# nyu-systems/Grendel-GS

Measured on AMD Instinct MI355X. Metric: training iters/sec (fwd+bwd), higher is better.
Workload: dtype f32

## Files before the change

grendel-gs_amd/csrc/composite.hip:

```cpp
#include "common.h"

namespace {

constexpr float LOG2E = 1.4426950408889634f;
constexpr float ALPHA_MIN = 1.0f / 255.0f;
constexpr float T_STOP = 0.0001f;

__device__ unsigned long long g_walked[2];

#ifdef GSR_STATS
__device__ unsigned long long g_stats[8];
#define GSR_STAT(i, v) do { const unsigned long long sv__ = (unsigned long long)(v); if (lane == 0) atomicAdd(&g_stats[i], sv__); } while (0)
#else
#define GSR_STAT(i, v) do { } while (0)
#endif

struct Entry {
    float x, y;
    float a2, b2, c2;
    float o;
    bool relevant;
};

#ifndef GSR_NO_LOG2O
#define GSR_LOG2O 1
#endif
__device__ __forceinline__ float entry_exponent(const float4 q0, const float4 q1, float dx, float dy) {
#ifdef GSR_LOG2O
    return fmaf(fmaf(q0.z, dx, q0.w * dy), dx, fmaf(q1.x * dy, dy, q1.y));
#else
    return (q0.z * dx + q0.w * dy) * dx + q1.x * dy * dy;
#endif
}
__device__ __forceinline__ float entry_alpha_raw(const float4 q1, float pe) {
#ifdef GSR_LOG2O
    return __builtin_amdgcn_exp2f(pe);
#else
    return q1.y * __builtin_amdgcn_exp2f(pe);
#endif
}
__device__ __forceinline__ bool entry_power_ok(const float4 q1, float pe) {
#ifdef GSR_LOG2O
    return pe <= q1.y;
#else
    return pe <= 0.f;
#endif
}

__device__ __forceinline__ float entry_opacity_term(float o) {
#ifdef GSR_LOG2O
    return __log2f(o);
#else
    return o;
#endif
}

__device__ __forceinline__ Entry load_entry(bool have, uint32_t id, const float2 *__restrict__ means2D,
                                            const float4 *__restrict__ conic_opacity, float qx0, float qy0) {
    Entry e;
    e.x = e.y = e.a2 = e.b2 = e.c2 = e.o = 0.f;
    e.relevant = false;
    if (have) {
        const float2 xy = means2D[id];
        const float4 co = conic_opacity[id];
        e.x = xy.x;
        e.y = xy.y;
        e.a2 = -0.5f * LOG2E * co.x;
        e.b2 = -LOG2E * co.y;
        e.c2 = -0.5f * LOG2E * co.z;
        e.o = entry_opacity_term(co.w);
        e.relevant = gsr_can_touch_box(xy, co, qx0, qy0, qx0 + 7.0f, qy0 + 7.0f);
    }
    return e;
}


typedef float v2f __attribute__((ext_vector_type(2)));
constexpr int PREC = 20;
struct PairRec {
    v2f x, y, a2, b2, c2, o, r, g, b;
};
__device__ __forceinline__ void pair_store(float *__restrict__ slab, int pos, const Entry &e, float r, float g, float b) {
    float *rec = slab + (pos >> 1) * PREC + (pos & 1);
    rec[0] = e.x;  rec[2] = e.y;  rec[4] = e.a2;  rec[6] = e.b2;  rec[8] = e.c2;
    rec[10] = e.o; rec[12] = r;   rec[14] = g;    rec[16] = b;
}
__device__ __forceinline__ void pair_store_last(float *__restrict__ slab, int pos, int last) {
    slab[(pos >> 1) * PREC + 18 + (pos & 1)] = __int_as_float(last);
}
__device__ __forceinline__ PairRec pair_load_last(const float *__restrict__ slab, int pair, int &la, int &lb) {
    const float4 *q = reinterpret_cast<const float4 *>(slab + pair * PREC);
    const float4 q0 = q[0], q1 = q[1], q2 = q[2], q3 = q[3], q4 = q[4];
    PairRec p;
    p.x = v2f{q0.x, q0.y};  p.y = v2f{q0.z, q0.w};  p.a2 = v2f{q1.x, q1.y};  p.b2 = v2f{q1.z, q1.w};
    p.c2 = v2f{q2.x, q2.y}; p.o = v2f{q2.z, q2.w};  p.r = v2f{q3.x, q3.y};   p.g = v2f{q3.z, q3.w};
    p.b = v2f{q4.x, q4.y};
    la = __float_as_int(q4.z);
    lb = __float_as_int(q4.w);
    asm("" : "+v"(la), "+v"(lb));
    return p;
}
#ifdef GSR_LOG2O
#define GSR_PAD_O (-__builtin_inff())
#else
#define GSR_PAD_O 0.f
#endif
__device__ __forceinline__ PairRec pair_load(const float *__restrict__ slab, int pair) {
    const float4 *q = reinterpret_cast<const float4 *>(slab + pair * PREC);
    const float4 q0 = q[0], q1 = q[1], q2 = q[2], q3 = q[3];
    const float2 q4 = *reinterpret_cast<const float2 *>(q + 4);
    PairRec p;
    p.x = v2f{q0.x, q0.y};  p.y = v2f{q0.z, q0.w};  p.a2 = v2f{q1.x, q1.y};  p.b2 = v2f{q1.z, q1.w};
    p.c2 = v2f{q2.x, q2.y}; p.o = v2f{q2.z, q2.w};  p.r = v2f{q3.x, q3.y};   p.g = v2f{q3.z, q3.w};
    p.b = v2f{q4.x, q4.y};
    return p;
}
__device__ __forceinline__ v2f pair_exponent(const PairRec &p, float pxf, float pyf) {
    const v2f dx = p.x - pxf, dy = p.y - pyf;
    return __builtin_elementwise_fma(__builtin_elementwise_fma(p.a2, dx, p.b2 * dy), dx,
                                     __builtin_elementwise_fma(p.c2 * dy, dy, p.o));
}

__device__ __forceinline__ int composite_tile_of_block(const int2 *__restrict__ ranges, int gx, int tiles) {
    const int2 hull = ranges[tiles];
    const int gy = tiles / gx;
    if (hull.x < 0 || hull.y > gy || hull.x >= hull.y) return gsr_xcd_span_of_block(blockIdx.x, tiles);
    return gsr_xcd_span_of_block_band(blockIdx.x, tiles, hull.x * gx, (hull.y - hull.x) * gx);
}

struct RawEntry {
    float2 xy;
    float4 co;
    float r, g, b;
};
__device__ __forceinline__ RawEntry load_raw(bool have, uint32_t id, const float2 *__restrict__ means2D,
                                             const float4 *__restrict__ conic_opacity, const float *__restrict__ rgb) {
    RawEntry e;
    e.xy = make_float2(0.f, 0.f);
    e.co = make_float4(0.f, 0.f, 0.f, 0.f);
    e.r = e.g = e.b = 0.f;
    if (have) {
        e.xy = means2D[id];
        e.co = conic_opacity[id];
        e.r = rgb[3 * (size_t)id];
        e.g = rgb[3 * (size_t)id + 1];
        e.b = rgb[3 * (size_t)id + 2];
    }
    return e;
}

#ifndef GSR_SEG_LEN
#define GSR_SEG_LEN 256
#endif
#ifndef GSR_SEG_MAXJ
#define GSR_SEG_MAXJ 16
#endif
constexpr int SEG_LEN = GSR_SEG_LEN;
constexpr int SEG_MAXJ = GSR_SEG_MAXJ;
static_assert(SEG_LEN % 64 == 0 && (SEG_LEN & (SEG_LEN - 1)) == 0 && SEG_MAXJ <= 31,
              "segment geometry: K8 finds boundaries with c & (SEG_LEN - 1), so SEG_LEN is a power of two");
constexpr int SEG_WORKERS = 1024;
constexpr int SEG_SLOT_FLOATS = 7 * 256;
struct SegWs {
    uint32_t *hdr;
    uint32_t *queue;
    int32_t *seg_slot;
    float *ckpt;
    uint32_t cap;
};
__host__ __device__ inline size_t seg_ws_bytes(int tiles, uint32_t cap) {
    return 64 + sizeof(uint32_t) * (size_t)cap + sizeof(int32_t) * (size_t)tiles * SEG_MAXJ + sizeof(float) * SEG_SLOT_FLOATS * (size_t)cap;
}
inline SegWs seg_ws_of(void *ws, int tiles, uint32_t cap) {
    SegWs w{};
    if (!ws) return w;
    char *b = reinterpret_cast<char *>(ws);
    w.hdr = reinterpret_cast<uint32_t *>(b);
    w.queue = reinterpret_cast<uint32_t *>(b + 64);
    w.seg_slot = reinterpret_cast<int32_t *>(b + 64 + sizeof(uint32_t) * (size_t)cap);
    w.ckpt = reinterpret_cast<float *>(b + 64 + sizeof(uint32_t) * (size_t)cap + sizeof(int32_t) * (size_t)tiles * SEG_MAXJ);
    w.cap = cap;
    return w;
}
constexpr uint32_t SEG_CAP = 8192;

__device__ __forceinline__ int k8_checkpoint(const SegWs &seg, int *s_slot, int tile, int c, int lane,
                                                       int wave, float T, float c0, float c1, float c2) {
    const int j = c / SEG_LEN - 1;
    int slot = 0;
    if (lane == 0) {
        int v = atomicCAS(&s_slot[j], -1, -2);
        if (v == -1) {
            const uint32_t k = atomicAdd(seg.hdr, 1u);
            v = k < seg.cap ? (int)k : -3;
            if (v >= 0) {
                seg.queue[k] = (uint32_t)tile * 32u + (uint32_t)(j + 1);
                seg.seg_slot[(size_t)tile * SEG_MAXJ + j] = v;
            }
            __hip_atomic_store(&s_slot[j], v, __ATOMIC_RELEASE, __HIP_MEMORY_SCOPE_WORKGROUP);
        } else {
            while (v == -2) v = __hip_atomic_load(&s_slot[j], __ATOMIC_ACQUIRE, __HIP_MEMORY_SCOPE_WORKGROUP);
        }
        slot = v;
    }
    slot = __builtin_amdgcn_readfirstlane(slot);
    if (slot >= 0) {
        float *ck = seg.ckpt + (size_t)slot * SEG_SLOT_FLOATS + wave * 64 + lane;
        ck[0] = T;
        ck[256] = c0;
        ck[512] = c1;
        ck[768] = c2;
    }
    return slot;
}

template <bool SEG, bool BAND>
__global__ void __launch_bounds__(256, SEG ? 6 : (BAND ? 7 : 8))
composite_forward_kernel(int W, int H, int gx, const int2 *__restrict__ ranges,
                         const uint32_t *__restrict__ point_list, const float2 *__restrict__ means2D,
                         const float4 *__restrict__ conic_opacity, const float *__restrict__ rgb,
                         const uint8_t *__restrict__ compute_locally, const float *__restrict__ bg,
                         float *__restrict__ out_color, float *__restrict__ final_T, int32_t *__restrict__ n_contrib,
                         const SegWs seg, int band_first, int band_tiles, uint4 *__restrict__ zero16,
                         size_t zero16_n) {
    const size_t HW = (size_t)H * W;
    for (size_t i = (size_t)blockIdx.x * 256 + threadIdx.x; i < zero16_n; i += (size_t)gridDim.x * 256)
        zero16[i] = make_uint4(0u, 0u, 0u, 0u);
    int tile;
    bool idle = false;
    if (BAND) {
        if (band_first < 0) {
            const int gy = (H + GSR_BLOCK_Y - 1) / GSR_BLOCK_Y;
            int2 hull = ranges[gx * gy];
            if (hull.x < 0 || hull.y > gy || hull.x >= hull.y) hull = make_int2(0, 0);
            band_first = hull.x * gx;
            band_tiles = min((hull.y - hull.x) * gx, band_tiles);
            idle = (int)blockIdx.x >= band_tiles;
        }
        tile = band_first + (idle ? 0 : gsr_xcd_span_of_block(blockIdx.x, band_tiles));
    } else {
        tile = composite_tile_of_block(ranges, gx, (int)gridDim.x);
    }
    auto clear_outside = [&]() {
        if (!BAND) return;
        const size_t n0 = (size_t)min(H, (band_first / gx) * GSR_BLOCK_Y) * W;
        const size_t p1 = (size_t)min(H, ((band_first + band_tiles) / gx) * GSR_BLOCK_Y) * W;
        const size_t nout = n0 + (HW - p1);
        for (size_t i = (size_t)blockIdx.x * 256 + threadIdx.x; i < nout; i += (size_t)gridDim.x * 256) {
            const size_t q = i < n0 ? i : p1 + (i - n0);
            out_color[q] = 0.f;
            out_color[HW + q] = 0.f;
            out_color[2 * HW + q] = 0.f;
            final_T[q] = 1.f;
            n_contrib[q] = 0;
        }
    };
    if (idle) {
        clear_outside();
        return;
    }
    const int lane = threadIdx.x & 63, wave = threadIdx.x >> 6;
    const int tx = tile % gx, ty = tile / gx;
    const int qx0 = tx * GSR_BLOCK_X + (wave & 1) * 8, qy0 = ty * GSR_BLOCK_Y + (wave >> 1) * 8;
    const int px = qx0 + (lane & 7), py = qy0 + (lane >> 3);
    const bool inside = px < W && py < H;
    const size_t pid = (size_t)py * W + px;

    if (!compute_locally[tile]) {
        if (inside) {
            out_color[pid] = 0.f;
            out_color[HW + pid] = 0.f;
            out_color[2 * HW + pid] = 0.f;
            final_T[pid] = 1.f;
            n_contrib[pid] = 0;
        }
        clear_outside();
        return;
    }
    const int2 range = ranges[tile];
    const int n = range.y - range.x;
    const float pxf = (float)px, pyf = (float)py;

    float T = 1.0f, C0 = 0.f, C1 = 0.f, C2 = 0.f;
    int last = 0;
    bool done = !inside;
    __shared__ __attribute__((aligned(16))) float slab[4][32 * PREC];
    __shared__ int s_walk[2];
    __shared__ int s_slot[SEG_MAXJ];
    if (threadIdx.x < 2) s_walk[threadIdx.x] = 0;
    if (SEG && threadIdx.x < SEG_MAXJ) {
        s_slot[threadIdx.x] = -1;
        if (seg.seg_slot) seg.seg_slot[(size_t)tile * SEG_MAXJ + threadIdx.x] = -1;
    }
    __syncthreads();
    v2f A0 = {0.f, 0.f}, A1 = {0.f, 0.f}, A2 = {0.f, 0.f};
    v2f B0 = {0.f, 0.f}, B1 = {0.f, 0.f}, B2 = {0.f, 0.f};
    int nstored = 0;
    float *wslab = slab[wave];
    int walked = 0;

    for (int c = 0; c < n; c += 64) {
        if (__all(done)) break;
        if (SEG && seg.seg_slot && c > 0 && (c & (SEG_LEN - 1)) == 0 && c <= SEG_LEN * SEG_MAXJ) {
            if (k8_checkpoint(seg, s_slot, tile, c, lane, wave, T, B0.x + B0.y, B1.x + B1.y, B2.x + B2.y) >= 0) {
                B0 = B1 = B2 = v2f{0.f, 0.f};
                nstored = c / SEG_LEN;
            }
        }
        walked = c + 64;
        const bool have = c + lane < n;
        const uint32_t id = have ? point_list[range.x + c + lane] : 0u;
        const Entry e = load_entry(have, id, means2D, conic_opacity, (float)qx0, (float)qy0);
        float r = 0.f, g = 0.f, b = 0.f;
        if (e.relevant) {
            r = rgb[3 * (size_t)id];
            g = rgb[3 * (size_t)id + 1];
            b = rgb[3 * (size_t)id + 2];
        }
        unsigned long long m = __ballot(e.relevant);
        GSR_STAT(0, __popcll(__ballot(have)));
        GSR_STAT(1, __popcll(m));
        const int nrel = __popcll(m);
#ifdef GSR_ABL_K8_MASKWALK
        if (e.relevant) pair_store(wslab, __popcll(m & ((1ull << lane) - 1ull)), e, r, g, b);
        {
            const int pad = (-nrel) & 3, slot = nrel + lane / 9;
            if (lane < 9 * pad) wslab[(slot >> 1) * PREC + 2 * (lane % 9) + (slot & 1)] = 0.f;
        }
#else
        if (e.relevant) {
            const int pos = __popcll(m & ((1ull << lane) - 1ull));
            pair_store(wslab, pos, e, r, g, b);
            pair_store_last(wslab, pos, c + lane + 1);
        }
        {
            const int pad = (-nrel) & 3, slot = nrel + lane / 10, f = lane % 10;
            if (lane < 10 * pad) wslab[(slot >> 1) * PREC + 2 * f + (slot & 1)] = f == 5 ? GSR_PAD_O : 0.f;
        }
#endif
        for (int p0 = 0; p0 < nrel; p0 += 4) {
            float al[4];
            bool ok[4];
            int kk[4];
            v2f cr[2], cg[2], cb[2];
#pragma unroll
            for (int h = 0; h < 2; h++) {
#ifdef GSR_ABL_K8_MASKWALK
                const PairRec pr = pair_load(wslab, (p0 >> 1) + h);
#else
                const PairRec pr = pair_load_last(wslab, (p0 >> 1) + h, kk[2 * h], kk[2 * h + 1]);
#endif
                const v2f pe = pair_exponent(pr, pxf, pyf);
                cr[h] = pr.r;
                cg[h] = pr.g;
                cb[h] = pr.b;
#pragma unroll
                for (int u = 0; u < 2; u++) {
#ifdef GSR_ABL_K8_MASKWALK
                    const bool live = m != 0;
                    kk[2 * h + u] = c + (live ? __builtin_ctzll(m) : 0) + 1;
                    m &= m - 1;
#else
                    const bool live = true;
#endif
                    const float pe1 = u ? pe.y : pe.x, lo = u ? pr.o.y : pr.o.x;
                    al[2 * h + u] = fminf(0.99f, __builtin_amdgcn_exp2f(pe1));
                    ok[2 * h + u] = live && pe1 <= lo && al[2 * h + u] >= ALPHA_MIN;
                }
            }
            float wv[4];
#pragma unroll
            for (int u = 0; u < 4; u++) {
                const float w0 = al[u] * T;
                const float test_T = T - w0;
                const bool take = !done && ok[u];
                const bool stop = take && __float_as_int(test_T) < __float_as_int(T_STOP);
                done = done || stop;
                const bool blend = take && !stop;
                wv[u] = blend ? w0 : 0.f;
                T = blend ? test_T : T;
                last = blend ? kk[u] : last;
            }
#pragma unroll
            for (int h = 0; h < 2; h++) {
                const v2f w2 = {wv[2 * h], wv[2 * h + 1]};
                A0 = __builtin_elementwise_fma(cr[h], w2, A0);
                A1 = __builtin_elementwise_fma(cg[h], w2, A1);
                A2 = __builtin_elementwise_fma(cb[h], w2, A2);
                if (SEG) {
                    B0 = __builtin_elementwise_fma(cr[h], w2, B0);
                    B1 = __builtin_elementwise_fma(cg[h], w2, B1);
                    B2 = __builtin_elementwise_fma(cb[h], w2, B2);
                }
            }
            if (__all(done)) break;
        }
    }
    if (lane == 0) {
        atomicMax(&s_walk[0], walked < n ? walked : n);
        if (atomicAdd(&s_walk[1], 1) == 3) atomicAdd(&g_walked[0], (unsigned long long)s_walk[0]);
    }
    C0 = A0.x + A0.y;
    C1 = A1.x + A1.y;
    C2 = A2.x + A2.y;
    if (SEG && nstored > 0) {
        float r0 = B0.x + B0.y, r1 = B1.x + B1.y, r2 = B2.x + B2.y;
        for (int j = nstored - 1; j >= 0; j--) {
            float *ck = seg.ckpt + (size_t)s_slot[j] * SEG_SLOT_FLOATS + wave * 64 + lane;
            ck[1024] = r0;
            ck[1280] = r1;
            ck[1536] = r2;
            r0 += ck[256];
            r1 += ck[512];
            r2 += ck[768];
        }
    }
    if (inside) {
        out_color[pid] = C0 + T * bg[0];
        out_color[HW + pid] = C1 + T * bg[1];
        out_color[2 * HW + pid] = C2 + T * bg[2];
        final_T[pid] = T;
        n_contrib[pid] = last;
    }
    clear_outside();
}

typedef float f32x4 __attribute__((ext_vector_type(4)));

constexpr int MB = 8;
constexpr int MSTR = 66;

__device__ __forceinline__ void
composite_backward_segment(const int tile, const int sidx, int W, int H, int gx, const int2 *__restrict__ ranges,
                           const uint32_t *__restrict__ point_list, const float2 *__restrict__ means2D,
                           const float4 *__restrict__ conic_opacity, const float *__restrict__ rgb,
                           const uint8_t *__restrict__ compute_locally, const float *__restrict__ bg,
                           const float *__restrict__ final_T, const int32_t *__restrict__ n_contrib,
                           const float *__restrict__ dL_dpixels, double *__restrict__ dL_record,
                           const SegWs &seg, uint8_t *__restrict__ touched) {
    if (!compute_locally[tile]) return;
    const int lane = threadIdx.x & 63, wave = threadIdx.x >> 6;
    const int tx = tile % gx, ty = tile / gx;
    const int qx0 = tx * GSR_BLOCK_X + (wave & 1) * 8, qy0 = ty * GSR_BLOCK_Y + (wave >> 1) * 8;
    const int px = qx0 + (lane & 7), py = qy0 + (lane >> 3);
    const bool inside = px < W && py < H;
    const size_t pid = (size_t)py * W + px;
    const size_t HW = (size_t)H * W;
    const int2 range = ranges[tile];
    const float pxf = (float)px, pyf = (float)py;

    const int c_lo = sidx * SEG_LEN;
    int end_slot = -1;
    if (seg.seg_slot && sidx < SEG_MAXJ) end_slot = seg.seg_slot[(size_t)tile * SEG_MAXJ + sidx];
    const int c_hi = end_slot >= 0 ? c_lo + SEG_LEN : 0x7fffffff;
    const float T_final = inside ? final_T[pid] : 0.f;
    const int last = inside ? n_contrib[pid] : 0;
    float g0 = 0.f, g1 = 0.f, g2 = 0.f;
    if (inside) {
        g0 = dL_dpixels[pid];
        g1 = dL_dpixels[HW + pid];
        g2 = dL_dpixels[2 * HW + pid];
    }
    const float tb = T_final * (bg[0] * g0 + bg[1] * g1 + bg[2] * g2);
    const float ddelx_dx = 0.5f * W, ddely_dy = 0.5f * H;

    __shared__ float2 smat[4][MB * MSTR];
    __shared__ float sacc[4][64 * 9];
    __shared__ __attribute__((aligned(16))) float slab[4][32 * PREC];
    __shared__ float fslab[64 * 7];
    __shared__ float sout[64 * 10];
    __shared__ int s_wmax[4];
    int wmax = min(last, c_hi);
#pragma unroll
    for (int d = 32; d >= 1; d >>= 1) wmax = max(wmax, __shfl_xor(wmax, d, 64));
    if (wmax <= c_lo) wmax = 0;
    if (lane == 0) s_wmax[wave] = wmax;
    for (int i = threadIdx.x; i < 4 * 64 * 9; i += 256) (&sacc[0][0])[i] = 0.f;
    __syncthreads();
    const int bmax = max(max(s_wmax[0], s_wmax[1]), max(s_wmax[2], s_wmax[3]));
    if (bmax == 0) return;
    if (threadIdx.x == 0) atomicAdd(&g_walked[1], (unsigned long long)(bmax - c_lo));
    int wbest = 0;
#pragma unroll
    for (int w = 1; w < 4; w++)
        if (s_wmax[w] > s_wmax[wbest]) wbest = w;

    const int kq = lane >> 4, j = lane & 15;
    float Bop[16];
    {
        const bool isg = j >= 6 && j < 9;
        const float xa = (j == 0 || j == 2 || j == 5) ? 1.f : 0.f, xb1 = (j == 1 || j == 4) ? 1.f : 0.f, xc = j == 3 ? 1.f : 0.f;
        const float ya = (j == 0 || j == 1 || j == 3) ? 1.f : 0.f, yb1 = (j == 2 || j == 4) ? 1.f : 0.f, yc = j == 5 ? 1.f : 0.f;
        const float xl = (float)((wave & 1) * 8 + kq);
        float X[2];
#pragma unroll
        for (int h = 0; h < 2; h++) {
            const float x = xl + 4.f * h;
            X[h] = fmaf(x, fmaf(xc, x, xb1), xa);
        }
        const int gx0 = qx0 + kq;
        const int cx0 = min(gx0, W - 1), cx1 = min(gx0 + 4, W - 1);
        const float *gb = dL_dpixels + (size_t)(isg ? j - 6 : 0) * HW;
        float G[16];
#pragma unroll
        for (int t = 0; t < 16; t++) G[t] = 0.f;
        if (isg) {
#pragma unroll
            for (int t = 0; t < 16; t++) G[t] = gb[(size_t)min(qy0 + (t >> 1), H - 1) * W + ((t & 1) ? cx1 : cx0)];
        }
#pragma unroll
        for (int t = 0; t < 16; t++) {
            const float y = (float)((wave >> 1) * 8 + (t >> 1));
            const float Y = fmaf(y, fmaf(yc, y, yb1), ya);
            const bool inb = ((t & 1) ? gx0 + 4 : gx0) < W && qy0 + (t >> 1) < H;
            Bop[t] = isg ? (inb ? G[t] : 0.f) : X[t & 1] * Y;
        }
    }
    const float *arow = reinterpret_cast<const float *>(&smat[wave][(j & 7) * MSTR + kq]) + (j >> 3);
    const bool my_cols = kq < 2 ? j < 6 : (j >= 6 && j < 9);
    float *wslab = slab[wave];

    float T = T_final;
    float rho = 0.f;
    if (end_slot >= 0 && last > c_hi) {
        const float *ck = seg.ckpt + (size_t)end_slot * SEG_SLOT_FLOATS + wave * 64 + lane;
        T = ck[0];
        rho = (ck[1024] * g0 + ck[1280] * g1 + ck[1536] * g2) * __builtin_amdgcn_rcpf(T);
    }

    const int c0 = ((bmax - 1) / 64) * 64;
    uint32_t id_cur = (c0 + lane < wmax) ? point_list[range.x + c0 + lane] : 0u;
    uint32_t id_nxt = (c0 >= c_lo + 64 && c0 - 64 + lane < wmax) ? point_list[range.x + c0 - 64 + lane] : 0u;
    RawEntry raw = load_raw(c0 + lane < wmax, id_cur, means2D, conic_opacity, rgb);

    for (int c = c0; c >= c_lo; c -= 64) {
        float *acc_tab = sacc[wave];
        const bool have_nxt = c >= c_lo + 64 && c - 64 + lane < wmax;
        const RawEntry raw_nxt = load_raw(have_nxt, id_nxt, means2D, conic_opacity, rgb);
        const uint32_t id_nxt2 = (c >= c_lo + 128 && c - 128 + lane < wmax) ? point_list[range.x + c - 128 + lane] : 0u;
        if (c < wmax) {
            const bool have = c + lane < wmax;
            Entry e;
            e.x = raw.xy.x;
            e.y = raw.xy.y;
            e.a2 = -0.5f * LOG2E * raw.co.x;
            e.b2 = -LOG2E * raw.co.y;
            e.c2 = -0.5f * LOG2E * raw.co.z;
            e.o = entry_opacity_term(raw.co.w);
            e.relevant = have && gsr_can_touch_box(raw.xy, raw.co, (float)qx0, (float)qy0, (float)qx0 + 7.0f, (float)qy0 + 7.0f);
            unsigned long long m = __ballot(e.relevant);
            GSR_STAT(0, __popcll(__ballot(have)));
            GSR_STAT(1, __popcll(m));
            GSR_STAT(6, 1);
            if (e.relevant) pair_store(wslab, __popcll((m >> lane) >> 1), e, raw.r, raw.g, raw.b);
            if (wave == wbest) {
                float *fe = &fslab[7 * lane];
                fe[0] = e.x;  fe[1] = e.y;  fe[2] = e.a2;  fe[3] = e.b2;  fe[4] = e.c2;
                fe[5] = __uint_as_float(id_cur);
                fe[6] = raw.co.w;
            }
            unsigned long long sk = 0ull;
            auto contract_batch = [&](int filled) {
                __builtin_amdgcn_wave_barrier();
                f32x4 acc = {0.f, 0.f, 0.f, 0.f}, acc1 = {0.f, 0.f, 0.f, 0.f};
#pragma unroll
                for (int t = 0; t < 16; t += 2) {
                    acc = __builtin_amdgcn_mfma_f32_16x16x4f32(arow[8 * t], Bop[t], acc, 0, 0, 0);
                    acc1 = __builtin_amdgcn_mfma_f32_16x16x4f32(arow[8 * t + 8], Bop[t + 1], acc1, 0, 0, 0);
                }
                acc += acc1;
                const uint32_t sk4 = (kq & 1) ? (uint32_t)(sk >> 32) : (uint32_t)sk;
#pragma unroll
                for (int r4 = 0; r4 < 4; r4++) {
                    const int slot = 4 * (kq & 1) + r4;
                    if (slot < filled && my_cols) acc_tab[(int)((sk4 >> (8 * r4)) & 0xffu) * 9 + j] = acc[r4];
                }
                GSR_STAT(5, 1);
                __builtin_amdgcn_wave_barrier();
                sk = 0ull;
            };
            int s = 0;
            for (int pi = 0; m; pi++) {
                const int ka = 63 - __builtin_clzll(m);
                m &= ~(1ull << ka);
                const bool two = m != 0ull;
                const int kb = two ? 63 - __builtin_clzll(m) : ka;
                m &= ~(1ull << kb);
                const PairRec pr = pair_load(wslab, pi);
                const v2f pe = pair_exponent(pr, pxf, pyf);
                const float aar = __builtin_amdgcn_exp2f(pe.x), bar = __builtin_amdgcn_exp2f(pe.y);
                const float aal = fminf(0.99f, aar), bal = fminf(0.99f, bar);
                const bool atake = (c + ka + 1 <= last) && pe.x <= pr.o.x && aal >= ALPHA_MIN;
                const bool btake = two && (c + kb + 1 <= last) && pe.y <= pr.o.y && bal >= ALPHA_MIN;
                const v2f cg = __builtin_elementwise_fma(pr.b, v2f{g2, g2}, __builtin_elementwise_fma(pr.g, v2f{g1, g1}, pr.r * g0));
                GSR_STAT(2, two ? 2 : 1);
                GSR_STAT(3, (__builtin_amdgcn_ballot_w64(atake) != 0ull) + (__builtin_amdgcn_ballot_w64(btake) != 0ull));
                GSR_STAT(4, __popcll(__builtin_amdgcn_ballot_w64(atake)) + __popcll(__builtin_amdgcn_ballot_w64(btake)));
                const v2f qa = {atake ? aar : 0.f, atake ? aal : 0.f};
                const v2f qb = {btake ? bar : 0.f, btake ? bal : 0.f};
                const v2f inv = {__builtin_amdgcn_rcpf(1.f - qa.y), __builtin_amdgcn_rcpf(1.f - qb.y)};
                const v2f tbi = inv * tb;
                {
                    const float Tn = T * inv.x;
                    const float dot = cg.x - rho;
                    const float da = fmaf(dot, Tn, -tbi.x);
                    const v2f qw = qa * v2f{da, Tn};
                    smat[wave][s * MSTR + lane] = make_float2(qw.x, qw.y);
                    rho = fmaf(qa.y, dot, rho);
                    T = Tn;
                }
                sk |= (unsigned long long)ka << (8 * s);
                s++;
                if (two) {
                    const float Tn = T * inv.y;
                    const float dot = cg.y - rho;
                    const float da = fmaf(dot, Tn, -tbi.y);
                    const v2f qw = qb * v2f{da, Tn};
                    smat[wave][s * MSTR + lane] = make_float2(qw.x, qw.y);
                    rho = fmaf(qb.y, dot, rho);
                    T = Tn;
                    sk |= (unsigned long long)kb << (8 * s);
                    s++;
                }
                if (s == MB) {
                    contract_batch(MB);
                    s = 0;
                }
            }
            if (s > 0) contract_batch(s);
        }
        __syncthreads();
        if (wave == ((c >> 6) & 3)) {
            const float tx0 = (float)(tx * GSR_BLOCK_X), ty0 = (float)(ty * GSR_BLOCK_Y);
            const int e9 = 9 * lane;
            float Sv[9];
#pragma unroll
            for (int v = 0; v < 9; v++) Sv[v] = (sacc[0][e9 + v] + sacc[1][e9 + v]) + (sacc[2][e9 + v] + sacc[3][e9 + v]);
            const float *fe = &fslab[7 * lane];
            const float ex = fe[0] - tx0, ey = fe[1] - ty0;
            const float cA = fe[2] * (-2.0f / LOG2E), cB = fe[3] * (-1.0f / LOG2E), cC = fe[4] * (-2.0f / LOG2E);
            const float A0 = Sv[0], Ax = Sv[1], Ay = Sv[2];
            const float Mx = fmaf(ex, A0, -Ax), My = fmaf(ey, A0, -Ay);
            float o[9];
            o[0] = -(cA * Mx + cB * My) * ddelx_dx;
            o[1] = -(cB * Mx + cC * My) * ddely_dy;
            o[2] = Sv[6];
            o[3] = Sv[7];
            o[4] = Sv[8];
            o[5] = -0.5f * (fmaf(fmaf(ex, A0, -2.f * Ax), ex, Sv[3]));
            o[6] = -(fmaf(ex, My, -ey * Ax) + Sv[4]);
            o[7] = -0.5f * (fmaf(fmaf(ey, A0, -2.f * Ay), ey, Sv[5]));
            o[8] = A0 == 0.f ? 0.f : A0 / fe[6];
            const bool live = c + lane < bmax;
            float *so = &sout[10 * lane];
#pragma unroll
            for (int v = 0; v < 9; v++) so[v] = live ? o[v] : 0.f;
            so[9] = fe[5];
        }
        __syncthreads();
#pragma unroll
        for (int r = 0; r < 3; r++) {
            const int idx = threadIdx.x + 256 * r;
            const int e = idx / 9, col = idx - 9 * e;
            if (idx < 576) {
                const float val = sout[10 * e + col];
#ifndef GSR_ABL_NOATOMIC
                if (val != 0.f) {
                    const uint32_t id = __float_as_uint(sout[10 * e + 9]);
                    atomicAdd(dL_record + 9 * (size_t)id + col, (double)val);
                    if (touched) touched[id] = 1;
                }
#else
                asm volatile("" ::"v"(val));
#endif
            }
        }
#pragma unroll
        for (int i = 0; i < 9; i++) acc_tab[64 * i + lane] = 0.f;
        raw = raw_nxt;
        id_cur = id_nxt;
        id_nxt = id_nxt2;
    }
}

__global__ void __launch_bounds__(256, 4)
composite_backward_kernel(int W, int H, int gx, int tiles, const int2 *__restrict__ ranges,
                          const uint32_t *__restrict__ point_list, const float2 *__restrict__ means2D,
                          const float4 *__restrict__ conic_opacity, const float *__restrict__ rgb,
                          const uint8_t *__restrict__ compute_locally, const float *__restrict__ bg,
                          const float *__restrict__ final_T, const int32_t *__restrict__ n_contrib,
                          const float *__restrict__ dL_dpixels, double *__restrict__ dL_record,
                          const SegWs seg, int band_first, int band_tiles, uint8_t *__restrict__ touched) {
    const int nstatic = band_tiles > 0 ? band_tiles : tiles;
    const bool worker = (int)blockIdx.x >= nstatic;
    if (band_first < 0 && band_tiles > 0) {
        const int gy = tiles / gx;
        int2 hull = ranges[tiles];
        if (hull.x < 0 || hull.y > gy || hull.x >= hull.y) hull = make_int2(0, 0);
        band_first = hull.x * gx;
        band_tiles = min((hull.y - hull.x) * gx, band_tiles);
        if (!worker && (int)blockIdx.x >= band_tiles) return;
    }
    __shared__ uint32_t s_item;
    const uint32_t count = worker ? min(seg.hdr[0], seg.cap) : 0u;
    for (;;) {
        int tile, sidx = 0;
        if (worker) {
            __syncthreads();
            if (threadIdx.x == 0) s_item = atomicAdd(&seg.hdr[1], 1u);
            __syncthreads();
            const uint32_t t = s_item;
            if (t >= count) return;
            const uint32_t item = seg.queue[t];
            tile = (int)(item >> 5);
            sidx = (int)(item & 31u);
        } else {
            tile = band_tiles > 0 ? band_first + gsr_xcd_span_of_block(blockIdx.x, band_tiles)
                                  : composite_tile_of_block(ranges, gx, tiles);
        }
        composite_backward_segment(tile, sidx, W, H, gx, ranges, point_list, means2D, conic_opacity, rgb,
                                   compute_locally, bg, final_T, n_contrib, dL_dpixels, dL_record, seg, touched);
        if (!worker) return;
    }
}

}

extern "C" int gsr_composite_walked(unsigned long long *out2, int reset) {
    if (!out2) return GSR_EINVAL;
    GSR_HIP(hipMemcpyFromSymbol(out2, HIP_SYMBOL(g_walked), sizeof(unsigned long long) * 2));
    if (reset) {
        const unsigned long long z[2] = {0ull, 0ull};
        GSR_HIP(hipMemcpyToSymbol(HIP_SYMBOL(g_walked), z, sizeof(z)));
    }
    return 0;
}

#ifdef GSR_STATS
extern "C" int gsr_debug_stats(unsigned long long *out8, int reset) {
    if (hipMemcpyFromSymbol(out8, HIP_SYMBOL(g_stats), sizeof(unsigned long long) * 8) != hipSuccess) return -1;
    if (reset) {
        unsigned long long z[8] = {0, 0, 0, 0, 0, 0, 0, 0};
        if (hipMemcpyToSymbol(HIP_SYMBOL(g_stats), z, sizeof(z)) != hipSuccess) return -1;
    }
    return 0;
}
#endif

size_t gsr_composite_seg_bytes(int W, int H) {
    const int gx = (W + GSR_BLOCK_X - 1) / GSR_BLOCK_X, gy = (H + GSR_BLOCK_Y - 1) / GSR_BLOCK_Y;
    return seg_ws_bytes(gx * gy, SEG_CAP);
}

struct BandGrid {
    bool band;
    int band_first;
    int band_tiles;
};
static BandGrid band_grid_of(int row_lo, int row_hi, int gx, int gy) {
    const bool dyn = row_lo == -1 && row_hi > 0 && row_hi <= gy;
    const bool band = dyn || (row_lo >= 0 && row_lo < row_hi && row_hi <= gy && !(row_lo == 0 && row_hi == gy));
    return {band, dyn ? -1 : band ? row_lo * gx : 0, dyn ? row_hi * gx : band ? (row_hi - row_lo) * gx : 0};
}

int gsr_launch_composite_forward(int P, int W, int H, const int32_t *ranges, const uint32_t *point_list,
                                 const float *means2D, const float *conic_opacity, const float *rgb,
                                 const uint8_t *compute_locally, const float *bg, float *out_color, float *final_T,
                                 int32_t *n_contrib, void *seg_ws, size_t seg_bytes, int row_lo, int row_hi,
                                 void *zero_ptr, size_t zero_bytes, hipStream_t stream) {
    (void)P;
    if (zero_bytes && (!zero_ptr || ((uintptr_t)zero_ptr & 15) || (zero_bytes & 3))) return GSR_EINVAL;
    const size_t zero16_n = zero_bytes / 16;
    if (zero_bytes & 15)
        GSR_HIP(hipMemsetAsync(reinterpret_cast<char *>(zero_ptr) + zero16_n * 16, 0, zero_bytes & 15, stream));
    const int gx = (W + GSR_BLOCK_X - 1) / GSR_BLOCK_X, gy = (H + GSR_BLOCK_Y - 1) / GSR_BLOCK_Y;
    const BandGrid b = band_grid_of(row_lo, row_hi, gx, gy);
    if (seg_ws && seg_bytes < seg_ws_bytes(gx * gy, SEG_CAP)) return GSR_ENOSPACE;
    const SegWs seg = seg_ws_of(seg_ws, gx * gy, SEG_CAP);
    if (seg_ws) GSR_HIP(hipMemsetAsync(seg_ws, 0, 64, stream));
    auto launch = [&](auto kern) {
        hipLaunchKernelGGL(kern, dim3(b.band ? b.band_tiles : gx * gy), dim3(256), 0, stream, W, H, gx,
                           reinterpret_cast<const int2 *>(ranges), point_list, reinterpret_cast<const float2 *>(means2D),
                           reinterpret_cast<const float4 *>(conic_opacity), rgb, compute_locally, bg, out_color, final_T,
                           n_contrib, seg, b.band_first, b.band_tiles, reinterpret_cast<uint4 *>(zero_ptr), zero16_n);
    };
    if (seg_ws && b.band) launch(composite_forward_kernel<true, true>);
    else if (seg_ws) launch(composite_forward_kernel<true, false>);
    else if (b.band) launch(composite_forward_kernel<false, true>);
    else launch(composite_forward_kernel<false, false>);
    GSR_LAUNCH_CHECK();
    return 0;
}

__global__ void record_from_f64_kernel(const double *__restrict__ acc, float *__restrict__ rec, size_t n) {
    const size_t i = (size_t)blockIdx.x * blockDim.x + threadIdx.x;
    if (i < n) rec[i] = (float)acc[i];
}

__global__ void record_from_f64_touched_kernel(const double *__restrict__ acc, float *__restrict__ rec,
                                               const uint8_t *__restrict__ touched, int P) {
    const int i = (int)(blockIdx.x * blockDim.x + threadIdx.x);
    if (i >= P || !touched[i]) return;
    const double *a = acc + 9 * (size_t)i;
    float *r = rec + 9 * (size_t)i;
    double v[9];
#pragma unroll
    for (int k = 0; k < 9; k++) v[k] = a[k];
#pragma unroll
    for (int k = 0; k < 9; k++) r[k] = (float)v[k];
}

int gsr_launch_composite_backward(int P, int W, int H, const int32_t *ranges, const uint32_t *point_list,
                                  const float *means2D, const float *conic_opacity, const float *rgb,
                                  const uint8_t *compute_locally, const float *bg, const float *final_T,
                                  const int32_t *n_contrib, const float *dL_dpixels, float *dL_record,
                                  const float *out_color, void *seg_ws, size_t seg_bytes, int row_lo, int row_hi,
                                  int record_is_zero, double *acc64, uint8_t *touched, hipStream_t stream) {
    if (!record_is_zero) {
        touched = nullptr;
        GSR_HIP(hipMemsetAsync(acc64, 0, sizeof(double) * 9 * (size_t)P, stream));
    }
    if (P == 0) return 0;
    const int gx = (W + GSR_BLOCK_X - 1) / GSR_BLOCK_X, gy = (H + GSR_BLOCK_Y - 1) / GSR_BLOCK_Y;
    const BandGrid b = band_grid_of(row_lo, row_hi, gx, gy);
    if (seg_ws && (seg_bytes < seg_ws_bytes(gx * gy, SEG_CAP) || !out_color)) return GSR_EINVAL;
    const SegWs seg = seg_ws_of(seg_ws, gx * gy, SEG_CAP);
    if (seg_ws) GSR_HIP(hipMemsetAsync(reinterpret_cast<char *>(seg_ws) + sizeof(uint32_t), 0, sizeof(uint32_t), stream));
    const dim3 grid((b.band ? b.band_tiles : gx * gy) + (seg_ws ? SEG_WORKERS : 0));
    hipLaunchKernelGGL(composite_backward_kernel, grid, dim3(256), 0, stream, W, H, gx, gx * gy,
                       reinterpret_cast<const int2 *>(ranges), point_list, reinterpret_cast<const float2 *>(means2D),
                       reinterpret_cast<const float4 *>(conic_opacity), rgb, compute_locally, bg, final_T, n_contrib,
                       dL_dpixels, acc64, seg, b.band_first, b.band_tiles, touched);
    GSR_LAUNCH_CHECK();
    if (touched)
        hipLaunchKernelGGL(record_from_f64_touched_kernel, dim3((unsigned)((P + 255) / 256)), dim3(256), 0, stream,
                           acc64, dL_record, touched, P);
    else
        hipLaunchKernelGGL(record_from_f64_kernel, dim3((unsigned)((9 * (size_t)P + 255) / 256)), dim3(256), 0, stream,
                           acc64, dL_record, 9 * (size_t)P);
    GSR_LAUNCH_CHECK();
    return 0;
}
```

Baseline: 808.0.

## Replace mask-driven backward walk with dense pair walk over compacted relevant entries

Each relevant entry's contribution index is now stored alongside its pair record, and the backward walk iterates directly over the compacted relevant list in fixed batches of eight. It no longer walks a bitmask and skips entries one by one. Accumulator rows for the MFMA scatter are derived from the stored indices rather than a packed slot-key word. This aims to remove branchy per-entry mask scanning and key packing, at the cost of extra shared-memory stores and loads for the index fields plus padding of odd pair counts.

```diff
diff --git a/grendel-gs_amd/csrc/composite.hip b/grendel-gs_amd/csrc/composite.hip
--- a/grendel-gs_amd/csrc/composite.hip
+++ b/grendel-gs_amd/csrc/composite.hip
@@ -429,6 +429,7 @@
 
 constexpr int MB = 8;
 constexpr int MSTR = 66;
+[[maybe_unused]] constexpr int K10_NO_POS = 0x7fffffff;
 
 __device__ __forceinline__ void
 composite_backward_segment(const int tile, const int sidx, int W, int H, int gx, const int2 *__restrict__ ranges,
@@ -552,13 +553,25 @@
             GSR_STAT(0, __popcll(__ballot(have)));
             GSR_STAT(1, __popcll(m));
             GSR_STAT(6, 1);
+#ifdef GSR_ABL_K10_MASKWALK
             if (e.relevant) pair_store(wslab, __popcll((m >> lane) >> 1), e, raw.r, raw.g, raw.b);
+#else
+            const int nrel = __popcll(m);
+            if (e.relevant) {
+                const int pos = __popcll((m >> lane) >> 1);
+                pair_store(wslab, pos, e, raw.r, raw.g, raw.b);
+                pair_store_last(wslab, pos, c + lane + 1);
+            }
+            if ((nrel & 1) && lane < 10)
+                wslab[(nrel >> 1) * PREC + 2 * lane + 1] = lane == 5 ? GSR_PAD_O : lane == 9 ? __int_as_float(K10_NO_POS) : 0.f;
+#endif
             if (wave == wbest) {
                 float *fe = &fslab[7 * lane];
                 fe[0] = e.x;  fe[1] = e.y;  fe[2] = e.a2;  fe[3] = e.b2;  fe[4] = e.c2;
                 fe[5] = __uint_as_float(id_cur);
                 fe[6] = raw.co.w;
             }
+#ifdef GSR_ABL_K10_MASKWALK
             unsigned long long sk = 0ull;
             auto contract_batch = [&](int filled) {
                 __builtin_amdgcn_wave_barrier();
@@ -628,6 +641,90 @@
                 }
             }
             if (s > 0) contract_batch(s);
+#else
+            auto contract_batch = [&](int b, int filled) {
+                __builtin_amdgcn_wave_barrier();
+                const float *pw = wslab + (4 * b + 2 * (kq & 1)) * PREC + 18;
+                float2 w01 = *reinterpret_cast<const float2 *>(pw), w23 = *reinterpret_cast<const float2 *>(pw + PREC);
+                asm("" : "+v"(w01.x), "+v"(w01.y), "+v"(w23.x), "+v"(w23.y));
+                f32x4 acc = {0.f, 0.f, 0.f, 0.f}, acc1 = {0.f, 0.f, 0.f, 0.f};
+#pragma unroll
+                for (int t = 0; t < 16; t += 2) {
+                    acc = __builtin_amdgcn_mfma_f32_16x16x4f32(arow[8 * t], Bop[t], acc, 0, 0, 0);
+                    acc1 = __builtin_amdgcn_mfma_f32_16x16x4f32(arow[8 * t + 8], Bop[t + 1], acc1, 0, 0, 0);
+                }
+                acc += acc1;
+                const int row[4] = {__float_as_int(w01.x) - (c + 1), __float_as_int(w01.y) - (c + 1),
+                                    __float_as_int(w23.x) - (c + 1), __float_as_int(w23.y) - (c + 1)};
+#pragma unroll
+                for (int r4 = 0; r4 < 4; r4++) {
+                    const int slot = 4 * (kq & 1) + r4;
+                    if (slot < filled && my_cols) acc_tab[row[r4] * 9 + j] = acc[r4];
+                }
+                GSR_STAT(5, 1);
+                __builtin_amdgcn_wave_barrier();
+            };
+            auto walk_pair = [&](const float *recs, int rp, int pi, float2 *mrow) {
+                int la, lb;
+                const PairRec pr = pair_load_last(recs, rp, la, lb);
+                const v2f pe = pair_exponent(pr, pxf, pyf);
+                const float aar = __builtin_amdgcn_exp2f(pe.x), bar = __builtin_amdgcn_exp2f(pe.y);
+                const float aal = fminf(0.99f, aar), bal = fminf(0.99f, bar);
+                const bool atake = la <= last && pe.x <= pr.o.x && aal >= ALPHA_MIN;
+                const bool btake = lb <= last && pe.y <= pr.o.y && bal >= ALPHA_MIN;
+                const v2f cg = __builtin_elementwise_fma(pr.b, v2f{g2, g2}, __builtin_elementwise_fma(pr.g, v2f{g1, g1}, pr.r * g0));
+                GSR_STAT(2, min(2, nrel - 2 * pi));
+                GSR_STAT(3, (__builtin_amdgcn_ballot_w64(atake) != 0ull) + (__builtin_amdgcn_ballot_w64(btake) != 0ull));
+                GSR_STAT(4, __popcll(__builtin_amdgcn_ballot_w64(atake)) + __popcll(__builtin_amdgcn_ballot_w64(btake)));
+                const v2f qa = {atake ? aar : 0.f, atake ? aal : 0.f};
+                const v2f qb = {btake ? bar : 0.f, btake ? bal : 0.f};
+                const v2f inv = {__builtin_amdgcn_rcpf(1.f - qa.y), __builtin_amdgcn_rcpf(1.f - qb.y)};
+                const v2f tbi = inv * tb;
+                {
+                    const float Tn = T * inv.x;
+                    const float dot = cg.x - rho;
+                    const float da = fmaf(dot, Tn, -tbi.x);
+                    const v2f qw = qa * v2f{da, Tn};
+                    mrow[0] = make_float2(qw.x, qw.y);
+                    rho = fmaf(qa.y, dot, rho);
+                    T = Tn;
+                }
+                {
+                    const float Tn = T * inv.y;
+                    const float dot = cg.y - rho;
+                    const float da = fmaf(dot, Tn, -tbi.y);
+                    const v2f qw = qb * v2f{da, Tn};
+                    mrow[MSTR] = make_float2(qw.x, qw.y);
+                    rho = fmaf(qb.y, dot, rho);
+                    T = Tn;
+                }
+            };
+#ifdef GSR_ABL_K10_SLOTCOUNT
+            int s = 0;
+            for (int pi = 0; pi < (nrel + 1) >> 1; pi++) {
+                walk_pair(wslab, pi, pi, &smat[wave][s * MSTR + lane]);
+                s += 2;
+                if (s == MB) {
+                    contract_batch(pi >> 2, nrel - 8 * (pi >> 2));
+                    s = 0;
+                }
+            }
+            if (s > 0) contract_batch(nrel >> 3, nrel & 7);
+#else
+            for (int b = 0; 8 * b < nrel; b++) {
+                const int filled = nrel - 8 * b;
+                const int np = min(MB / 2, (filled + 1) >> 1);
+                float2 *const mrow = &smat[wave][lane];
+                const float *const brec = wslab + 4 * b * PREC;
+#pragma unroll
+                for (int k = 0; k < MB / 2; k++) {
+                    if (k >= np) break;
+                    walk_pair(brec, k, 4 * b + k, mrow + 2 * k * MSTR);
+                }
+                contract_batch(b, filled);
+            }
+#endif
+#endif
         }
         __syncthreads();
         if (wave == ((c >> 6) & 3)) {
```

New measurement: 820.6, median of 6. 1.02x the previous value.
